# microsoft/Sora

Measured on AMD Instinct MI355X. Metric: IQ Msamples/s through 802.11a 54 Mbps RX PHY, higher is better.
Workload: dtype int16 IQ / u8 path metrics

## Files before the change

### sora_amd/csrc/k_scan.hip

```cpp
#include <hip/hip_runtime.h>
#include "kernels.h"

namespace sora {

constexpr uint32_t kRing = 512;
__shared__ uint32_t s_ring[kRing];

#ifdef SORA_SCAN_PROBE
__device__ unsigned long long g_scan_probe[16];
#define PROBE_DECL() long long _pa[8] = {0, 0, 0, 0, 0, 0, 0, 0}; unsigned _pn[8] = {0, 0, 0, 0, 0, 0, 0, 0}
#define PROBE_T0() const long long _t0 = clock64()
#define PROBE_ADD(i) do { _pa[i] += clock64() - _t0; _pn[i]++; } while (0)
#define PROBE_T(n) const long long n = clock64()
#define PROBE_A(n, i) do { _pa[i] += clock64() - n; _pn[i]++; } while (0)
#define PROBE_TK() const long long _tk = clock64()
#define PROBE_ADDK(i) do { _pa[i] += clock64() - _tk; _pn[i]++; \
    if (blockIdx.x == 0 && threadIdx.x == 0) for (int q = 0; q < 8; q++) { g_scan_probe[q] += (unsigned long long)_pa[q]; g_scan_probe[8 + q] += _pn[q]; } } while (0)
#else
#define PROBE_DECL()
#define PROBE_T0()
#define PROBE_ADD(i)
#define PROBE_T(n)
#define PROBE_A(n, i)
#define PROBE_TK()
#define PROBE_ADDK(i)
#endif

struct Acc4 { int reg; uint32_t Z; };
__device__ __forceinline__ void acc_clear(Acc4& a) { a.reg = 0; a.Z = 0; }
__device__ __forceinline__ void acc_push(Acc4& a, int d)
{
    const int e0 = __builtin_amdgcn_readfirstlane((int)a.Z);
    a.reg = (int)((unsigned)a.reg + (unsigned)d - (unsigned)e0);
    const uint32_t sh = (uint32_t)__builtin_amdgcn_update_dpp(0, (int)a.Z, 0x104, 0xF, 0xF, true);
    a.Z = (threadIdx.x & 12u) == 12u ? (uint32_t)d : sh;
}
__device__ __forceinline__ uint32_t group_scan(uint32_t t)
{
    t += (uint32_t)__builtin_amdgcn_update_dpp(0, (int)t, 0x114, 0xF, 0xF, true);
    t += (uint32_t)__builtin_amdgcn_update_dpp(0, (int)t, 0x118, 0xF, 0xF, true);
    t += (uint32_t)__builtin_amdgcn_update_dpp(0, (int)t, 0x142, 0xA, 0xF, false);
    return t;
}

__device__ __forceinline__ uint32_t group_scan64(uint32_t t)
{
    t += (uint32_t)__builtin_amdgcn_update_dpp(0, (int)t, 0x114, 0xF, 0xF, true);
    t += (uint32_t)__builtin_amdgcn_update_dpp(0, (int)t, 0x118, 0xF, 0xF, true);
    t += (uint32_t)__builtin_amdgcn_update_dpp(0, (int)t, 0x142, 0xA, 0xF, false);
    t += (uint32_t)__builtin_amdgcn_update_dpp(0, (int)t, 0x143, 0xC, 0xF, false);
    return t;
}
__device__ __forceinline__ uint32_t shift16(uint32_t v, uint32_t first)
{
    auto r16 = __builtin_amdgcn_permlane16_swap(v, v, false, false);
    auto r32 = __builtin_amdgcn_permlane32_swap(r16[1], r16[1], false, false);
    const uint32_t l = threadIdx.x;
    return l < 16u ? first : (l & 48u) == 32u ? r32[0] : r16[0];
}
__device__ __forceinline__ uint32_t compress4(uint64_t x)
{
    x = (x | (x >> 3)) & 0x0303030303030303ull;
    x = (x | (x >> 6)) & 0x000F000F000F000Full;
    x = (x | (x >> 12)) & 0x000000FF000000FFull;
    return (uint32_t)((x | (x >> 24)) & 0xFFFFull);
}

template <int CTRL> __device__ __forceinline__ unsigned sdpp(unsigned v) { return (unsigned)__builtin_amdgcn_update_dpp(0, (int)v, CTRL, 0xF, 0xF, true); }
__device__ __forceinline__ unsigned quad_sum(unsigned v) { v += sdpp<0xB1>(v); v += sdpp<0x4E>(v); return v; }
__device__ __forceinline__ unsigned row_sum(unsigned v) { v = quad_sum(v); v += sdpp<0x141>(v); v += sdpp<0x140>(v); return v; }
__device__ __forceinline__ unsigned other_row_even(unsigned v)
{
    auto r = __builtin_amdgcn_permlane16_swap(v, v, false, false);
    return r[0];
}
__device__ __forceinline__ int wave_sum(int v)
{
    unsigned u = row_sum((unsigned)v);
    auto r16 = __builtin_amdgcn_permlane16_swap(u, u, false, false);
    u = r16[0] + r16[1];
    auto r32 = __builtin_amdgcn_permlane32_swap(u, u, false, false);
    return (int)(r32[0] + r32[1]);
}
__device__ __forceinline__ unsigned wave_min(unsigned v)
{
    v = min(v, sdpp<0xB1>(v)); v = min(v, sdpp<0x4E>(v)); v = min(v, sdpp<0x141>(v)); v = min(v, sdpp<0x140>(v));
    auto r16 = __builtin_amdgcn_permlane16_swap(v, v, false, false);
    v = min(r16[0], r16[1]);
    auto r32 = __builtin_amdgcn_permlane32_swap(v, v, false, false);
    return min(r32[0], r32[1]);
}

__device__ __constant__ uint8_t kLtsSeq[64] = {
    0,1,0,0,1,1,0,1,0,1,0,0,0,0,0,1, 1,0,0,1,0,1,0,1,1,1,1,0,0,0,0,0,
    0,0,0,0,0,0,1,1,0,0,1,1,0,1,0,1, 1,1,1,1,1,0,0,1,1,0,1,0,1,1,1,1 };

__device__ __forceinline__ int carrier_bin(int k)
{
    if (k < 24) { int b = 38 + k; if (b >= 43) b++; if (b >= 57) b++; return b; }
    int b = 1 + (k - 24); if (b >= 7) b++; if (b >= 21) b++; return b;
}

struct ScanTabs { const short* uatan2; const uint32_t* rot; const uint8_t* demap; const uint16_t* deint; const uint32_t* tw64; const uint32_t* tw16; };
template <typename P> __device__ __forceinline__ P* uni_ptr(P* p)
{
    const uint64_t v = (uint64_t)(uintptr_t)p;
    const uint32_t lo = (uint32_t)__builtin_amdgcn_readfirstlane((int)(uint32_t)v), hi = (uint32_t)__builtin_amdgcn_readfirstlane((int)(uint32_t)(v >> 32));
    return (P*)(uintptr_t)(((uint64_t)hi << 32) | lo);
}
__device__ __forceinline__ Tables tables_of(const ScanTabs& b)
{
    Tables T = {};
    T.uatan2 = uni_ptr(b.uatan2); T.rot = uni_ptr(b.rot); T.demap = uni_ptr(b.demap); T.deint = uni_ptr(b.deint); T.tw64 = uni_ptr(b.tw64); T.tw16 = uni_ptr(b.tw16);
    return T;
}

struct SigOut { uint32_t ok, kbps, len, nsym, cr, nb; int cfo_comp, sfo_comp, cfo_tr, sfo_tr, cfo; };
__device__ __noinline__ SigOut header_section(ScanTabs tabs, uint32_t lts_start_, FrameCtx* fx_)
{
    const Tables T = tables_of(tabs);
    FrameCtx* fx = uni_ptr(fx_);
    const uint32_t lts_start = (uint32_t)__builtin_amdgcn_readfirstlane((int)lts_start_), sym_start = lts_start + 144u;
    __shared__ uint32_t s_a[64], s_b[64];
    __shared__ uint8_t  s_soft[64];
    const int lane = threadIdx.x, e = lane & 15;
    auto sync = []() { wave_lds_sync(); };
    const Fft64TwPk W = fft64_twiddles_pk(T, e);
    const int t2 = lane < 24 ? 2 * lane : 0;
    const int d0 = T.deint[t2], d1 = T.deint[t2 + 1];
    const cpx x1 = sra(unpack(s_ring[(lts_start + 8u + (uint32_t)lane) & (kRing - 1u)]), 1);
    const cpx x2 = unpack(s_ring[(lts_start + 72u + (uint32_t)lane) & (kRing - 1u)]);
    const cpx sg = sra(unpack(s_ring[(sym_start + 8u + (uint32_t)lane) & (kRing - 1u)]), 1);
    int re, im; conj_mul32(x2, x1, re, im);
    const int sum_re = __builtin_amdgcn_readfirstlane(wave_sum(re >> 5)), sum_im = __builtin_amdgcn_readfirstlane(wave_sum(im >> 5));
    const int arg = __builtin_amdgcn_readfirstlane(uatan2(T, sum_im, sum_re));
    const int cfo = arg >> 6;
    const cpx fc = rot_coeff(T, w16(lane * cfo));
    fx->freq[lane] = pack(fc);
    s_a[lane] = pack(mul_q15(x1, fc));
    s_b[lane] = pack(mul_q15(sg, fc));
    {
        uint32_t* const sf = (lane & 16) ? s_b : s_a;
        sync();
        const pcx xin[4] = { sf[e], sf[e + 16], sf[e + 32], sf[e + 48] };
        fft64_core_pk(xin, sf, e, W, sync);
    }
    const unsigned slot = __brev((unsigned)lane) >> 26;
    const cpx Yl = unpack(s_a[slot]), Ys = unpack(s_b[slot]);
    cpx eq = mk(0, 0);
    {
        uint32_t coef = 0;
        if (!(lane >= 28 && lane < 36)) {
            const int en = sqnorm(Yl) >> 8;
            const cpx L = mk(kLtsSeq[lane] ? 1600 : -1600, 0);
            int cre, cim; conj_mul32(L, Yl, cre, cim);
            int rre = 0, rim = 0;
            if (en != 0) { rre = cre / en; rim = cim / en; }
            coef = pack(mk(w16(rre), w16(rim)));
            int qr, qi; mul32(Ys, unpack(coef), qr, qi);
            eq = mk(w16(qr >> 8), w16(qi >> 8));
        }
        fx->chan[lane] = coef;
    }
    const cpx pc = mul_q15(eq, mk(0x7fff, 0));
    const uint32_t ppc = pack(pc);
    const cpx p43 = unpack((uint32_t)__builtin_amdgcn_readlane((int)ppc, 43)), p57 = unpack((uint32_t)__builtin_amdgcn_readlane((int)ppc, 57));
    const cpx p7 = unpack((uint32_t)__builtin_amdgcn_readlane((int)ppc, 7)), p21 = unpack((uint32_t)__builtin_amdgcn_readlane((int)ppc, 21));
    const int th1 = __builtin_amdgcn_readfirstlane(uatan2(T, p43.im, p43.re)), th2 = __builtin_amdgcn_readfirstlane(uatan2(T, p57.im, p57.re));
    const int th3 = __builtin_amdgcn_readfirstlane(uatan2(T, p7.im, p7.re)),   th4 = __builtin_amdgcn_readfirstlane(uatan2(T, -p21.im, -p21.re));
    const int avg = w16((th1 + th2 + th3 + th4) / 4);
    const int del = w16(((th3 - th1) / 28 + (th4 - th2) / 28) >> 1);
    const int cfo_tracker = w16(avg >> 2), sfo_tracker = w16(del >> 2);
    const int cfo_comp = w16(avg + cfo_tracker), sfo_comp = w16(del + sfo_tracker);
    {
        const int cidx = lane < 32 ? lane : lane - 64;
        const cpx r = mul_q15(pc, rot_coeff(T, w16(avg + cidx * del)));
        int v = r.re >> 4; v = min(max(v, -128), 127);
        s_soft[lane] = (uint8_t)((v >= -30) + (v >= -17) + (v >= -8) + (v >= 0) + (v >= 9) + (v >= 18) + (v >= 31));
    }
    sync();
    uint8_t sa = 0, sb = 0;
    if (lane < 24) { sa = s_soft[carrier_bin(d0)]; sb = s_soft[carrier_bin(d1)]; }
    auto rol6c = [](unsigned x, unsigned k) { return ((x << k) | (x >> (6u - k))) & 63u; };
    int selV[6], negV[6], n29V[6];
#pragma unroll
    for (int k = 0; k < 6; k++) {
        const unsigned n = k ? rol6c((unsigned)lane, (unsigned)k) : (unsigned)lane;
        const int cA = __popc(n & 0155) & 1, cB = __popc(n & 0117) & 1;
        selV[k] = (cA ^ cB) ? -1 : 0; negV[k] = cB ? -1 : 0; n29V[k] = cB ? 29 : 0;
    }
    unsigned m = (lane == 0) ? 0u : 0x30u;
    uint64_t dec[25];
    dec[0] = 0;
#pragma unroll
    for (int u = 1; u <= 24; u++) {
        const int ph = (u - 1) % 6, k = u % 6;
        const unsigned X = 32u >> ph;
        unsigned pm;
        if (ph == 0) { auto r = __builtin_amdgcn_permlane32_swap(m, m, false, false); pm = lane < 32 ? r[1] : r[0]; }
        else if (ph == 1) { auto r = __builtin_amdgcn_permlane16_swap(m, m, false, false); pm = (lane & 16) ? r[0] : r[1]; }
        else if (ph == 2) pm = sdpp<0x128>(m);
        else if (ph == 3) {
            const int t4 = __builtin_amdgcn_update_dpp(0, (int)m, 0x114, 0xF, 0xA, false);
            pm = (unsigned)__builtin_amdgcn_update_dpp(t4, (int)m, 0x104, 0xF, 0x5, false);
        }
        else if (ph == 4) pm = sdpp<0x4E>(m);
        else pm = sdpp<0xB1>(m);
        asm volatile("" : "+v"(pm));
        const bool own_hi = ((unsigned)lane & X) != 0u;
        const unsigned m0 = own_hi ? pm : m, m1 = own_hi ? m : pm;
        const int va = __builtin_amdgcn_readlane((int)sa, u - 1), vb = __builtin_amdgcn_readlane((int)sb, u - 1);
        const int P = 2 * va + 2 * vb, dQP = 14 - 4 * va;
        const int x = P + (selV[k] & dQP);
        const unsigned b0 = (unsigned)((x ^ negV[k]) + n29V[k]), b1 = 28u - b0;
        const unsigned c0 = (m0 + b0) & 0xFE, c1 = ((m1 + b1) & 0xFF) | 1;
        m = min(c0, c1);
        dec[u] = __ballot(m & 1);
        if ((u & 7) == 0) m = (m - (wave_min(m) & 0xFE)) & 0xFF;
    }
    const unsigned key = (m << 8) | ((unsigned)lane << 2);
    const unsigned kmin = (unsigned)__builtin_amdgcn_readfirstlane((int)wave_min(key));
    int pos = (int)((kmin >> 2) & 0x3F) | (int)(((kmin >> 8) & 1) << 6);
    uint32_t sig = 0;
#pragma unroll
    for (int b = 0; b < 24; b++) {
        sig |= (uint32_t)((pos >> 6) & 1) << (23 - b);
        pos = (pos >> 1) & 0x3F;
        const unsigned r = (unsigned)(23 - b) % 6u;
        const unsigned ln = r ? rol6c((unsigned)pos, 6u - r) : (unsigned)pos;
        pos |= (int)((dec[23 - b] >> ln) & 1) << 6;
    }
    sig = (uint32_t)__builtin_amdgcn_readfirstlane((int)sig) >> 6;
    bool ok = true;
    sig &= 0xFFFFFF;
    if (sig & 0xFC0010) ok = false;
    uint32_t par = (sig >> 16) ^ sig; par = (par >> 8) ^ par; par = (par >> 4) ^ par; par = (par >> 2) ^ par; par = (par >> 1) ^ par;
    if (par & 1) ok = false;
    uint32_t kbps = 0; int nd = 0, nb = 0, cr = 0;
    switch (sig & 0xF) {
    case 0x8: kbps = 48000; nd = 192; nb = 6; cr = 1; break;  case 0x9: kbps = 24000; nd = 96;  nb = 4; cr = 0; break;
    case 0xA: kbps = 12000; nd = 48;  nb = 2; cr = 0; break;  case 0xB: kbps = 6000;  nd = 24;  nb = 1; cr = 0; break;
    case 0xC: kbps = 54000; nd = 216; nb = 6; cr = 2; break;  case 0xD: kbps = 36000; nd = 144; nb = 4; cr = 2; break;
    case 0xE: kbps = 18000; nd = 72;  nb = 2; cr = 2; break;  case 0xF: kbps = 9000;  nd = 36;  nb = 1; cr = 2; break;
    default: ok = false; break;
    }
    const uint32_t len = (sig >> 5) & 0xFFF;
    if (len > 2500) ok = false;
    SigOut O;
    O.ok = ok ? 1u : 0u; O.kbps = kbps; O.len = len; O.cr = (uint32_t)cr; O.nb = (uint32_t)nb;
    O.nsym = ok ? (len * 8 + 16 + 6 + (uint32_t)nd - 1) / (uint32_t)nd : 0u;
    O.cfo_comp = cfo_comp; O.sfo_comp = sfo_comp; O.cfo_tr = cfo_tracker; O.sfo_tr = sfo_tracker; O.cfo = cfo;
    __threadfence_block();
    sync();
    return O;
}

constexpr uint32_t kContMagic = 0x534F5241u;
__device__ __noinline__ void cont_store(uint32_t* crec, uint32_t* consumed, uint32_t Hv, uint32_t Zr, uint32_t Zi, uint32_t Ze, int rr, int ri, int re,
                                        uint32_t sense_count, uint32_t high_count, int peak_corr, int peak_index, uint32_t dc_cnt, int sum_dc_re, int sum_dc_im,
                                        int dc_re, int dc_im, uint32_t at, uint32_t nfr)
{
    const int l = threadIdx.x;
    const uint32_t zr = (uint32_t)__shfl((int)Zr, 4 * (l & 3)), zi = (uint32_t)__shfl((int)Zi, 4 * (l & 3)), ze = (uint32_t)__shfl((int)Ze, 4 * (l & 3));
    const uint32_t hv = (uint32_t)__shfl((int)Hv, l & 15);
    uint32_t v = l < 16 ? hv : l < 20 ? zr : l < 24 ? zi : l < 28 ? ze : 0u;
    const uint32_t sc[16] = { (uint32_t)rr, (uint32_t)ri, (uint32_t)re, sense_count, high_count, (uint32_t)peak_corr, (uint32_t)peak_index, dc_cnt,
                              (uint32_t)sum_dc_re, (uint32_t)sum_dc_im, (uint32_t)dc_re, (uint32_t)dc_im, at, kContMagic, nfr, 0u };
#pragma unroll
    for (int k = 0; k < 16; k++) if (l == 28 + k) v = sc[k];
    crec[l] = v;
    if (l == 0) *consumed = at;
}
__device__ __noinline__ void cont_rows(const uint32_t* crec, uint32_t* nframes, FrameRow* rows, uint32_t written)
{
    const uint32_t n = (uint32_t)__builtin_amdgcn_readlane((int)crec[threadIdx.x], 42);
    if (threadIdx.x == 0) {
        *nframes = n;
        for (uint32_t k = n; k < written; k++) rows[k].valid = 0;
    }
}

__device__ __forceinline__ uint32_t div14(uint32_t x) { return (uint32_t)(((uint64_t)x * 0x92492493ull) >> 35); }
__device__ __forceinline__ uint32_t call_end(uint32_t burst_end) { return div14(burst_end + 13u) * 14u; }

__global__ void __launch_bounds__(64, 4) k_scan(ScanArgs A)
{
    const uint32_t cap_i = blockIdx.x;
    if (cap_i >= A.ncaps) return;
    const int lane = threadIdx.x;
    const CapDesc cd = A.caps[cap_i];
    const uint32_t* iq = A.iq + cd.offset;
    const uint32_t sh = A.str - 1u;
    const uint32_t NS = (cd.nsamples / (14u << sh)) * 14u;
    const Tables& T = A.T;
    const ScanTabs tabs = { T.uatan2, T.rot, T.demap, T.deint, T.tw64, T.tw16 };

    uint32_t n0 = 0, n1 = 0, n2 = 0, n3 = 0, r_lo = 0, r_hi = 0;
    auto issue = [&](uint32_t base) {
        const uint32_t i = base + (uint32_t)lane;
        n0 = i < NS ? iq[(size_t)i << sh] : 0u;
        n1 = i + 64u < NS ? iq[(size_t)(i + 64u) << sh] : 0u;
        n2 = i + 128u < NS ? iq[(size_t)(i + 128u) << sh] : 0u;
        n3 = i + 192u < NS ? iq[(size_t)(i + 192u) << sh] : 0u;
    };
    auto aim = [&](uint32_t at) { if (at < r_lo || at >= r_hi + 256u) { r_lo = r_hi = at; issue(at); } };
    auto fill = [&](uint32_t at, uint32_t len) {
        aim(at);
        while (at + len > r_hi) {
            const uint32_t w = r_hi + (uint32_t)lane;
            s_ring[w & (kRing - 1u)] = n0; s_ring[(w + 64u) & (kRing - 1u)] = n1; s_ring[(w + 128u) & (kRing - 1u)] = n2; s_ring[(w + 192u) & (kRing - 1u)] = n3;
            r_hi += 256u;
            if (r_hi - r_lo > kRing) r_lo = r_hi - kRing;
            issue(r_hi);
        }
    };
    issue(0);

    if (A.own_slots && A.slot_row) for (uint32_t i = (uint32_t)lane; i < cd.nslots; i += 64u) A.slot_row[cd.slot_base + i] = 0xFFFFFFFFu;
    if (cap_i == 0) {
        if (A.zero_a) for (uint32_t i = (uint32_t)lane; i < A.nzero_a; i += 64u) A.zero_a[i] = 0u;
        if (A.zero_b) for (uint32_t i = (uint32_t)lane; i < A.nzero_b; i += 64u) A.zero_b[i] = 0u;
    }
    const uint32_t chk0 = T.sts[lane & 15], chk1 = T.sts[16 + (lane & 15)], chk2 = T.sts[32 + (lane & 15)], chk3 = T.sts[48 + (lane & 15)];
    const uint32_t est_base = (uint32_t)(lane >> 2) * 16u + 4u * (uint32_t)(lane & 3);
    const uint32_t est0 = T.sts[est_base], est1 = T.sts[est_base + 1], est2 = T.sts[est_base + 2], est3 = T.sts[est_base + 3];

    uint32_t Hv = 0;
    Acc4 ac_re, ac_im, energy;
    uint32_t auto_count = 0, sense_count = 0, high_count = 0; int sync_high = 0, peak_corr = 0, peak_index = 0;
    uint32_t dc_cnt = 8; int sum_dc_re = 0, sum_dc_im = 0;
    int dc_re = 0, dc_im = 0;
    int cca_detected = 0;
    uint32_t frame_start = 0, nfr = 0;
    bool to_pending = false; uint32_t pend_end = 0;

    auto cs_reset = [&]() {
        Hv = 0;
        acc_clear(ac_re); acc_clear(ac_im); acc_clear(energy);
        auto_count = sense_count = high_count = 0; sync_high = 0; peak_corr = 0; peak_index = 0;
        dc_cnt = 8; sum_dc_re = sum_dc_im = 0;
    };
    cs_reset();

    const bool streaming = A.cont != nullptr;
    auto cont_save = [&](uint32_t at) {
        cont_store(A.cont + (size_t)cap_i * kContWords, A.consumed + cap_i, Hv, ac_re.Z, ac_im.Z, energy.Z, ac_re.reg, ac_im.reg, energy.reg, sense_count,
                high_count, peak_corr, peak_index,
                   dc_cnt, sum_dc_re, sum_dc_im, dc_re, dc_im, at << sh, nfr);
    };
    if (streaming) {
        if (lane == 0) A.consumed[cap_i] = 0;
        const uint32_t v = A.cont[(size_t)cap_i * kContWords + lane];
        if (lane == 42) A.cont[(size_t)cap_i * kContWords + lane] = 0;
        if ((uint32_t)__builtin_amdgcn_readlane((int)v, 41) == kContMagic) {
            auto sc = [&](int k) { return (uint32_t)__builtin_amdgcn_readlane((int)v, 28 + k); };
            Hv = (uint32_t)__shfl((int)v, lane & 15);
            ac_re.Z = (uint32_t)__shfl((int)v, 16 + ((lane & 15) >> 2)); ac_im.Z = (uint32_t)__shfl((int)v, 20 + ((lane & 15) >> 2));
                energy.Z = (uint32_t)__shfl((int)v, 24 + ((lane & 15) >> 2));
            ac_re.reg = (int)sc(0); ac_im.reg = (int)sc(1); energy.reg = (int)sc(2); sense_count = sc(3); high_count = sc(4); peak_corr = (int)sc(5); peak_index = (int)sc(6);
            dc_cnt = sc(7); sum_dc_re = (int)sc(8); sum_dc_im = (int)sc(9); dc_re = (int)sc(10); dc_im = (int)sc(11);
        }
    }

    uint32_t q_job = 0, nq = 0;
    auto flush_jobs = [&]() {
        if (nq == 0) return;
        const bool have = (uint32_t)lane < nq;
        const uint32_t cr = q_job >> 28, row = q_job & 0x0FFFFFFFu;
        const uint64_t m0 = __ballot(have && cr == 0u), m1 = __ballot(have && cr == 1u), m2 = __ballot(have && cr == 2u);
        const uint32_t cnt = lane == 0 ? (uint32_t)__popcll(m0) : lane == 1 ? (uint32_t)__popcll(m1) : (uint32_t)__popcll(m2);
        uint32_t base = 0;
        if (lane < 3 && cnt) base = atomicAdd(A.njobs + lane, cnt);
        const uint32_t b0 = (uint32_t)__builtin_amdgcn_readlane((int)base, 0), b1 = (uint32_t)__builtin_amdgcn_readlane((int)base, 1), b2 = (uint32_t)__builtin_amdgcn_readlane((int)base, 2);
        if (have) {
            const uint64_t mine = cr == 0u ? m0 : cr == 1u ? m1 : m2, below = ((uint64_t)1 << lane) - 1u;
            A.joblist[(size_t)cr * A.nrows + (cr == 0u ? b0 : cr == 1u ? b1 : b2) + (uint32_t)__popcll(mine & below)] = row;
        }
        nq = 0;
    };
    uint32_t s = 0;
    PROBE_DECL();
    PROBE_TK();
    auto ctx_of = [&](uint32_t k) { return A.fctx + (k < A.max_frames ? (size_t)cap_i * A.max_frames + k : (size_t)A.nrows + cap_i); };
    auto uni = [](int v) { return __builtin_amdgcn_readfirstlane(v); };

    for (;;) {
        PROBE_T(_tg);
        if (to_pending && s + 4u > pend_end) {
            to_pending = false; cca_detected = 0; cs_reset();
        }
        if (s + 4u > NS) break;
        if (!sync_high) {
            const bool plain = !to_pending && auto_count == 0;
            const uint32_t p = dc_cnt;
            uint32_t K = min(min((NS - s) >> 2, p + 9u), 16u);
            uint32_t jraise = 0xFFFFu, ce_raise = 0;
            if (to_pending) K = min(K, (pend_end - s) >> 2);
            else {
                jraise = sense_count >= 84u ? 0u : (84u - sense_count + 3u) / 4u - 1u;
                if (jraise < K) { const uint32_t be = s + 4u * jraise + 4u; ce_raise = call_end(be); K = min(K, jraise + 1u + ((ce_raise - be) >> 2)); }
            }
            if (streaming) {
                if (A.keep_queue) {
                    const uint32_t m = s % 140u;
                    if (m == 0u && plain) cont_save(s);
                    if (m) K = min(K, (143u - m) >> 2);
                } else {
                    const uint32_t m = s - div14(s) * 14u;
                    if (m == 0u && plain) cont_save(s);
                    const uint32_t j = (3u * (m >> 1)) % 7u;
                    K = min(K, j ? j : 7u);
                }
            }
            PROBE_A(_tg, 1);
            PROBE_T0();
            fill(s, 64u);
            const cpx x = unpack(s_ring[(s + (uint32_t)lane) & (kRing - 1u)]);
            int dcr = dc_re, dci = dc_im;
            if (p + 1u < K) {
                const unsigned hr = group_scan64(quad_sum((unsigned)(w16(x.re - dc_re) >> 5))), hi_ = group_scan64(quad_sum((unsigned)(w16(x.im - dc_im) >> 5)));
                const int sr = w16(sum_dc_re + __builtin_amdgcn_readlane((int)hr, (int)(4u * p))), si = w16(sum_dc_im + __builtin_amdgcn_readlane((int)hi_, (int)(4u * p)));
                const int d1r = w16(dc_re + (sr >> 2)), d1i = w16(dc_im + (si >> 2));
                const bool behind = (uint32_t)lane > 4u * p + 3u;
                dcr = behind ? d1r : dc_re; dci = behind ? d1i : dc_im;
            }
            const cpx pi = mk(w16(x.re - dcr), w16(x.im - dci));
            const cpx pii = sra(pi, 2);
            const uint32_t ppk = pack(pii);
            const uint32_t prev = shift16(ppk, Hv);
            int re, im; conj_mul32(pii, unpack(prev), re, im);
            unsigned vr = (unsigned)(re >> 4), vi = (unsigned)(im >> 4), ve = (unsigned)(sqnorm(pii) >> 4);
            vr = quad_sum(vr); vi = quad_sum(vi); ve = quad_sum(ve);
            const uint32_t Dr = group_scan64(quad_sum((unsigned)(pi.re >> 5))), Di = group_scan64(quad_sum((unsigned)(pi.im >> 5)));
            const uint32_t Rr = (uint32_t)ac_re.reg + group_scan64(vr - shift16(vr, ac_re.Z)), Ri = (uint32_t)ac_im.reg + group_scan64(vi - shift16(vi, ac_im.Z)),
                           Re = (uint32_t)energy.reg + group_scan64(ve - shift16(ve, energy.Z));
            const int iAuto_v = abs((int)Rr) + abs((int)Ri), iEnergy_v = (int)Re;
            const bool carrier = iEnergy_v > (int)A.thr && iAuto_v >= iEnergy_v - (iEnergy_v >> 3);
            const uint32_t hits = compress4((uint64_t)__ballot(carrier) & 0x1111111111111111ull) & ((1u << K) - 1u);
            const uint32_t a = min(auto_count, 3u);
            const uint32_t M = (hits << a) | ((1u << a) - 1u);
            const uint32_t run = M & (M >> 1) & (M >> 2) & (M >> 3);
            const bool est = run != 0;
            const uint32_t done = est ? (uint32_t)__builtin_ctz(run) + 4u - a : K;
            const uint32_t bits = (1u << done) - 1u;
            const uint32_t th = hits & bits;
            if (est) auto_count = 4;
            else {
                const uint32_t inv = ~th & bits;
                auto_count = inv ? done - 1u - (31u - (uint32_t)__builtin_clz(inv)) : min(auto_count + done, 4u);
            }
            if (!to_pending && jraise < min(th ? (uint32_t)__builtin_ctz(th) : done, done)) { to_pending = true; pend_end = ce_raise; }
            sense_count = th ? 4u * (done - 1u - (31u - (uint32_t)__builtin_clz(th))) : sense_count + 4u * done;
            {
                const int last = (int)(4u * (done - 1u));
                ac_re.reg = __builtin_amdgcn_readlane((int)Rr, last); ac_im.reg = __builtin_amdgcn_readlane((int)Ri, last); energy.reg = __builtin_amdgcn_readlane((int)Re, last);
                const uint32_t src = ((uint32_t)lane & 15u) + 4u * done;
                const int from_old = (int)(((uint32_t)lane & 48u) | (src & 15u)), from_new = (int)(src - 16u);
                const uint32_t fr = (uint32_t)__shfl((int)vr, from_new), fi = (uint32_t)__shfl((int)vi, from_new), fe = (uint32_t)__shfl((int)ve, from_new);
                const uint32_t fresh = (uint32_t)__shfl((int)ppk, from_new);
                if (done < 4u) {
                    const bool old = src < 16u;
                    const uint32_t kr = (uint32_t)__shfl((int)ac_re.Z, from_old), ki = (uint32_t)__shfl((int)ac_im.Z, from_old), ke = (uint32_t)__shfl((int)energy.Z, from_old);
                    const uint32_t keep = (uint32_t)__shfl((int)Hv, from_old);
                    ac_re.Z = old ? kr : fr; ac_im.Z = old ? ki : fi; energy.Z = old ? ke : fe; Hv = old ? keep : fresh;
                } else { ac_re.Z = fr; ac_im.Z = fi; energy.Z = fe; Hv = fresh; }
            }
            s += 4u * done;
            PROBE_ADD(3);
            if (est) {
                PROBE_T0();
                unsigned sr = 0, si = 0;
                {
                    const int q4 = 4 * (lane & 3);
                    const uint32_t h0 = (uint32_t)__shfl((int)Hv, q4), h1 = (uint32_t)__shfl((int)Hv, q4 + 1), h2 = (uint32_t)__shfl((int)Hv, q4 + 2), h3 = (uint32_t)__shfl((int)Hv, q4 + 3);
                    int cr_, ci_;
                    conj_mul32(unpack(est0), unpack(h0), cr_, ci_); sr += (unsigned)cr_; si += (unsigned)ci_;
                    conj_mul32(unpack(est1), unpack(h1), cr_, ci_); sr += (unsigned)cr_; si += (unsigned)ci_;
                    conj_mul32(unpack(est2), unpack(h2), cr_, ci_); sr += (unsigned)cr_; si += (unsigned)ci_;
                    conj_mul32(unpack(est3), unpack(h3), cr_, ci_); sr += (unsigned)cr_; si += (unsigned)ci_;
                }
                sr = quad_sum(sr); si = quad_sum(si);
                const int corr = abs((int)sr) + abs((int)si);
                int sum_corr = 0, best = 0, best_i = 0;
#pragma unroll
                for (int p = 0; p < 16; p++) {
                    const int cp = __builtin_amdgcn_readlane(corr, 4 * p);
                    if (cp > best) { best = cp; best_i = p; }
                    sum_corr += cp;
                }
                peak_corr = best; if (best > 0) peak_index = best_i;
                if (peak_corr > (sum_corr >> 3)) {
                    sync_high = 1; high_count = 0;
                    if (peak_index > 3) { high_count = (uint32_t)peak_index / 4; peak_index &= 3; }
                }
                PROBE_ADD(0);
            }
            const uint32_t ndc = done - (sync_high ? 1u : 0u);
            if (ndc > p) {
                const int at_p = __builtin_amdgcn_readlane((int)Dr, (int)(4u * p)), at_pi = __builtin_amdgcn_readlane((int)Di, (int)(4u * p));
                dc_re = w16(dc_re + (w16(sum_dc_re + at_p) >> 2)); dc_im = w16(dc_im + (w16(sum_dc_im + at_pi) >> 2));
                const uint32_t n1 = ndc - 1u - p;
                const int lastd = (int)(4u * (ndc - 1u));
                const int seg_re = w16(__builtin_amdgcn_readlane((int)Dr, lastd) - at_p), seg_im = w16(__builtin_amdgcn_readlane((int)Di, lastd) - at_pi);
                if (n1 == 8u) { dc_re = w16(dc_re + (seg_re >> 2)); dc_im = w16(dc_im + (seg_im >> 2)); sum_dc_re = sum_dc_im = 0; dc_cnt = 7; }
                else { sum_dc_re = seg_re; sum_dc_im = seg_im; dc_cnt = 7u - n1; }
            } else if (ndc) {
                const int lastd = (int)(4u * (ndc - 1u));
                sum_dc_re = w16(sum_dc_re + __builtin_amdgcn_readlane((int)Dr, lastd));
                sum_dc_im = w16(sum_dc_im + __builtin_amdgcn_readlane((int)Di, lastd));
                dc_cnt -= ndc;
            }
            continue;
        }

        {
            PROBE_T0();
            const uint32_t o = high_count & 3u;
            uint32_t Kn = min(16u - o, (NS - s) >> 2);
            if (to_pending) Kn = min(Kn, (pend_end - s) >> 2);
            fill(s, 64u);
            const cpx x = unpack(s_ring[(s + (uint32_t)lane - 4u * o) & (kRing - 1u)]);
            const cpx pi = mk(w16(x.re - dc_re), w16(x.im - dc_im));
            const uint32_t ppk = pack(sra(pi, 2));
            uint32_t hvr = Hv;
            if (o == 1u) hvr = sdpp<0x124>(Hv); else if (o == 2u) hvr = sdpp<0x128>(Hv); else if (o == 3u) hvr = sdpp<0x12C>(Hv);
            const uint32_t c = (uint32_t)lane < 4u * o ? hvr : ppk;
            const uint32_t pat = peak_index == 0 ? chk0 : peak_index == 1 ? chk1 : peak_index == 2 ? chk2 : chk3;
            int re, im; conj_mul32(unpack(pat), unpack(c), re, im);
            const unsigned ur = row_sum((unsigned)re), ui = row_sum((unsigned)im);
            unsigned dr = (unsigned)(pi.re >> 5), di = (unsigned)(pi.im >> 5);
            dr = quad_sum(dr); di = quad_sum(di);
            const uint32_t nchk = (o + Kn) >> 2;
            uint32_t taken = Kn;
#pragma unroll
            for (uint32_t r = 0; r < 4u; r++) {
                if (r < nchk && taken == Kn) {
                    const int corr = abs(__builtin_amdgcn_readlane((int)ur, 16 * (int)r)) + abs(__builtin_amdgcn_readlane((int)ui, 16 * (int)r));
                    if (corr < (peak_corr >> 1)) {
                        const uint32_t b = 4u * (r + 1u) - o - 1u;
                        taken = b + 1u;
                        if (high_count + taken > 8u) { cca_detected = 1; frame_start = s + 4u * b + 4u; }
                        else {
                            sync_high = 0; sense_count = 0;
                            sum_dc_re = w16(sum_dc_re + w16(__builtin_amdgcn_readlane((int)dr, 16 * (int)r + 12)));
                            sum_dc_im = w16(sum_dc_im + w16(__builtin_amdgcn_readlane((int)di, 16 * (int)r + 12)));
                            if (dc_cnt == 0) {
                                dc_re = w16(dc_re + (sum_dc_re >> 2)); dc_im = w16(dc_im + (sum_dc_im >> 2));
                                dc_cnt = 8; sum_dc_re = sum_dc_im = 0;
                            }
                            dc_cnt--;
                        }
                        if (taken == Kn) break;
                    } else if (corr > peak_corr) peak_corr = corr;
                }
            }
            high_count += taken;
            {
                const uint32_t src = ((uint32_t)lane & 15u) + 4u * taken;
                const uint32_t fresh = (uint32_t)__shfl((int)ppk, (int)((src - 16u + 4u * o) & 63u));
                if (taken < 4u) { const uint32_t keep = (uint32_t)__shfl((int)Hv, (int)(((uint32_t)lane & 48u) | (src & 15u))); Hv = src < 16u ? keep : fresh; }
                else Hv = fresh;
            }
            s += 4u * taken;
            PROBE_ADD(4);
        }
        if (!cca_detected) continue;

        const uint32_t lts_start = s, sym_start = s + 144u;
        if (sym_start + 80u > NS) break;
        PROBE_T(_tf);
        fill(lts_start, 224u);
        PROBE_A(_tf, 6);
        FrameCtx* const fx = ctx_of(nfr);
        PROBE_T(_ts);
        const SigOut so = header_section(tabs, lts_start, fx);
        const int r_cfo = uni(so.cfo);
        PROBE_A(_ts, 2);
        PROBE_T(_tc);
        const bool ok = uni((int)so.ok) != 0;
        const uint32_t r_nsym = ok ? (uint32_t)uni((int)so.nsym) : 0u, r_cr = ok ? (uint32_t)uni((int)so.cr) : 0u;
        const uint64_t ev = ok ? (uint64_t)sym_start + 80ull * (r_nsym + 1u) : (uint64_t)sym_start + 80ull;
        if (ev > NS) break;
        const uint32_t ce = call_end((uint32_t)ev), consumed_to = (uint32_t)ev + (((ce - (uint32_t)ev) >> 2) << 2);
        const uint32_t s_next = A.keep_queue ? consumed_to : ce;
        aim(s_next);
        {
            const bool has_row = nfr < A.max_frames;
            const uint32_t slot0 = cd.slot_base + sym_start / 80u;
            if (ok && has_row) {
                if ((uint32_t)lane == nq) q_job = (r_cr << 28) | (cap_i * A.max_frames + nfr);
                if (++nq == 64u) flush_jobs();
                if (A.slot_row) for (uint32_t sy = 1u + (uint32_t)lane; sy <= r_nsym; sy += 64u) A.slot_row[slot0 + sy] = cap_i * A.max_frames + nfr;
            }
            if (lane == 0 && has_row) {
                FrameRow row;
                row.capture = cap_i; row.start_sample = frame_start; row.end_sample = ok ? (uint32_t)ev : consumed_to;
                row.error_code = ok ? 0u : E_PLCP_HEADER_FAIL;
                row.rate_kbps = ok ? (uint32_t)uni((int)so.kbps) : 0u; row.length = (uint16_t)(ok ? (uint32_t)uni((int)so.len) : 0u); row.nsym = (uint16_t)r_nsym;
                row.code_rate = (uint16_t)r_cr; row.nbpsc = (uint16_t)(ok ? (uint32_t)uni((int)so.nb) : 0u); row.slot0 = slot0; row.crc32 = 0;
                row.cfo_est = (int16_t)r_cfo; row.cfo_comp = (int16_t)uni(so.cfo_comp); row.sfo_comp = (int16_t)uni(so.sfo_comp);
                row.cfo_tracker = (int16_t)uni(so.cfo_tr); row.sfo_tracker = (int16_t)uni(so.sfo_tr); row.valid = 1;
                row.data_start = sym_start; row.pad[0] = row.pad[1] = row.pad[2] = 0;
                A.frames[(size_t)cap_i * A.max_frames + nfr] = row;
            }
        }
        nfr++;
        s = s_next;
        to_pending = false; cca_detected = 0; cs_reset();
        PROBE_A(_tc, 7);
    }
    if (streaming && s == NS && !cca_detected && !sync_high && auto_count == 0 && !to_pending && (!A.keep_queue || s % 140u == 0u)) cont_save(s);
    flush_jobs();
    if (streaming) cont_rows(A.cont + (size_t)cap_i * kContWords, A.nframes + cap_i, A.frames + (size_t)cap_i * A.max_frames, min(nfr, A.max_frames));
    else if (lane == 0) A.nframes[cap_i] = nfr;
    PROBE_ADDK(5);
}

}

#ifdef SORA_SCAN_PROBE
extern "C" __attribute__((visibility("default"))) int sora_debug_scan_probe(unsigned long long* out, int reset)
{
    if (hipMemcpyFromSymbol(out, HIP_SYMBOL(sora::g_scan_probe), sizeof(unsigned long long) * 16) != hipSuccess) return -1;
    if (reset) { unsigned long long z[16] = {0}; (void)hipMemcpyToSymbol(HIP_SYMBOL(sora::g_scan_probe), z, sizeof(z)); }
    return 0;
}
#endif
```

Baseline: 55090.

## Restructure SIGNAL Viterbi ACS with packed branch metrics and table-driven selectors

```diff
diff --git a/sora_amd/csrc/k_scan.hip b/sora_amd/csrc/k_scan.hip
--- a/sora_amd/csrc/k_scan.hip
+++ b/sora_amd/csrc/k_scan.hip
@@ -115,6 +115,22 @@
     return T;
 }
 
+struct SigSel { uint32_t w[64][8]; };
+constexpr SigSel make_sig_sel()
+{
+    SigSel t = {};
+    for (unsigned p = 0; p < 64; p++)
+        for (unsigned k = 0; k < 6; k++) {
+            const unsigned n = k ? ((p << k) | (p >> (6u - k))) & 63u : p;
+            unsigned a = n & 0155u, b = n & 0117u, cA = 0, cB = 0;
+            for (; a; a >>= 1) cA ^= a & 1u;
+            for (; b; b >>= 1) cB ^= b & 1u;
+            t.w[p][k] = ((cA + 2u * cB) << 24) | 0x000C0C0Cu;
+        }
+    return t;
+}
+__device__ __constant__ const SigSel kSigSel = make_sig_sel();
+
 struct SigOut { uint32_t ok, kbps, len, nsym, cr, nb; int cfo_comp, sfo_comp, cfo_tr, sfo_tr, cfo; };
 __device__ __noinline__ SigOut header_section(ScanTabs tabs, uint32_t lts_start_, FrameCtx* fx_)
 {
@@ -128,6 +144,9 @@
     const Fft64TwPk W = fft64_twiddles_pk(T, e);
     const int t2 = lane < 24 ? 2 * lane : 0;
     const int d0 = T.deint[t2], d1 = T.deint[t2 + 1];
+    unsigned sel[6];
+#pragma unroll
+    for (int k = 0; k < 6; k++) sel[k] = kSigSel.w[lane][k];
     const cpx x1 = sra(unpack(s_ring[(lts_start + 8u + (uint32_t)lane) & (kRing - 1u)]), 1);
     const cpx x2 = unpack(s_ring[(lts_start + 72u + (uint32_t)lane) & (kRing - 1u)]);
     const cpx sg = sra(unpack(s_ring[(sym_start + 8u + (uint32_t)lane) & (kRing - 1u)]), 1);
@@ -181,56 +200,50 @@
     sync();
     uint8_t sa = 0, sb = 0;
     if (lane < 24) { sa = s_soft[carrier_bin(d0)]; sb = s_soft[carrier_bin(d1)]; }
-    auto rol6c = [](unsigned x, unsigned k) { return ((x << k) | (x >> (6u - k))) & 63u; };
-    int selV[6], negV[6], n29V[6];
-#pragma unroll
-    for (int k = 0; k < 6; k++) {
-        const unsigned n = k ? rol6c((unsigned)lane, (unsigned)k) : (unsigned)lane;
-        const int cA = __popc(n & 0155) & 1, cB = __popc(n & 0117) & 1;
-        selV[k] = (cA ^ cB) ? -1 : 0; negV[k] = cB ? -1 : 0; n29V[k] = cB ? 29 : 0;
-    }
-    unsigned m = (lane == 0) ? 0u : 0x30u;
+    const unsigned bmw = [&]() {
+        const unsigned P = 2u * sa + 2u * sb, Q = 14u - 2u * sa + 2u * sb;
+        return P | (Q << 8) | ((28u - Q) << 16) | ((28u - P) << 24);
+    }();
+    unsigned M = (lane == 0) ? 0u : 0x30u << 24;
     uint64_t dec[25];
-    dec[0] = 0;
+    bool last = false;
 #pragma unroll
     for (int u = 1; u <= 24; u++) {
         const int ph = (u - 1) % 6, k = u % 6;
-        const unsigned X = 32u >> ph;
-        unsigned pm;
-        if (ph == 0) { auto r = __builtin_amdgcn_permlane32_swap(m, m, false, false); pm = lane < 32 ? r[1] : r[0]; }
-        else if (ph == 1) { auto r = __builtin_amdgcn_permlane16_swap(m, m, false, false); pm = (lane & 16) ? r[0] : r[1]; }
-        else if (ph == 2) pm = sdpp<0x128>(m);
+        unsigned M0, M1;
+        if (ph == 0) { auto r = __builtin_amdgcn_permlane32_swap(M, M, false, false); M0 = r[0]; M1 = r[1]; }
+        else if (ph == 1) { auto r = __builtin_amdgcn_permlane16_swap(M, M, false, false); M0 = r[0]; M1 = r[1]; }
+        else if (ph == 2) {
+            M0 = (unsigned)__builtin_amdgcn_update_dpp((int)M, (int)M, 0x118, 0xF, 0xC, false);
+            M1 = (unsigned)__builtin_amdgcn_update_dpp((int)M, (int)M, 0x108, 0xF, 0x3, false);
+        }
         else if (ph == 3) {
-            const int t4 = __builtin_amdgcn_update_dpp(0, (int)m, 0x114, 0xF, 0xA, false);
-            pm = (unsigned)__builtin_amdgcn_update_dpp(t4, (int)m, 0x104, 0xF, 0x5, false);
-        }
-        else if (ph == 4) pm = sdpp<0x4E>(m);
-        else pm = sdpp<0xB1>(m);
-        asm volatile("" : "+v"(pm));
-        const bool own_hi = ((unsigned)lane & X) != 0u;
-        const unsigned m0 = own_hi ? pm : m, m1 = own_hi ? m : pm;
-        const int va = __builtin_amdgcn_readlane((int)sa, u - 1), vb = __builtin_amdgcn_readlane((int)sb, u - 1);
-        const int P = 2 * va + 2 * vb, dQP = 14 - 4 * va;
-        const int x = P + (selV[k] & dQP);
-        const unsigned b0 = (unsigned)((x ^ negV[k]) + n29V[k]), b1 = 28u - b0;
-        const unsigned c0 = (m0 + b0) & 0xFE, c1 = ((m1 + b1) & 0xFF) | 1;
-        m = min(c0, c1);
-        dec[u] = __ballot(m & 1);
-        if ((u & 7) == 0) m = (m - (wave_min(m) & 0xFE)) & 0xFF;
-    }
-    const unsigned key = (m << 8) | ((unsigned)lane << 2);
-    const unsigned kmin = (unsigned)__builtin_amdgcn_readfirstlane((int)wave_min(key));
-    int pos = (int)((kmin >> 2) & 0x3F) | (int)(((kmin >> 8) & 1) << 6);
+            M0 = (unsigned)__builtin_amdgcn_update_dpp((int)M, (int)M, 0x114, 0xF, 0xA, false);
+            M1 = (unsigned)__builtin_amdgcn_update_dpp((int)M, (int)M, 0x104, 0xF, 0x5, false);
+        }
+        else if (ph == 4) { M0 = sdpp<0x44>(M); M1 = sdpp<0xEE>(M); }
+        else { M0 = sdpp<0xA0>(M); M1 = sdpp<0xF5>(M); }
+        asm volatile("" : "+v"(M0), "+v"(M1));
+        const unsigned w = (unsigned)__builtin_amdgcn_readlane((int)bmw, u - 1);
+        const unsigned B0 = __builtin_amdgcn_perm(w, w, sel[k]);
+        const unsigned C0 = M0 + B0, C1 = M1 + ((28u << 24) - B0);
+        last = C1 < C0;
+        dec[u] = __ballot(last);
+        M = min(C0, C1);
+        if (u == 8 || u == 16) M -= wave_min(M);
+    }
+    const unsigned key = M | (last ? 1u << 24 : 0u) | (unsigned)lane;
+    unsigned L = (unsigned)__builtin_amdgcn_readfirstlane((int)wave_min(key)) & 63u;
     uint32_t sig = 0;
 #pragma unroll
-    for (int b = 0; b < 24; b++) {
-        sig |= (uint32_t)((pos >> 6) & 1) << (23 - b);
-        pos = (pos >> 1) & 0x3F;
-        const unsigned r = (unsigned)(23 - b) % 6u;
-        const unsigned ln = r ? rol6c((unsigned)pos, 6u - r) : (unsigned)pos;
-        pos |= (int)((dec[23 - b] >> ln) & 1) << 6;
-    }
-    sig = (uint32_t)__builtin_amdgcn_readfirstlane((int)sig) >> 6;
+    for (int g = 0; g < 3; g++) {
+#pragma unroll
+        for (int i = 0; i < 6; i++) {
+            const unsigned d = (unsigned)(dec[24 - 6 * g - i] >> L) & 1u;
+            L = (L & ~(1u << i)) | (d << i);
+        }
+        sig |= __brev(L) >> (14 + 6 * g);
+    }
     bool ok = true;
     sig &= 0xFFFFFF;
     if (sig & 0xFC0010) ok = false;
@@ -383,13 +396,14 @@
     PROBE_TK();
     auto ctx_of = [&](uint32_t k) { return A.fctx + (k < A.max_frames ? (size_t)cap_i * A.max_frames + k : (size_t)A.nrows + cap_i); };
     auto uni = [](int v) { return __builtin_amdgcn_readfirstlane(v); };
+    const uint32_t need = streaming ? 4u : 224u;
 
     for (;;) {
         PROBE_T(_tg);
         if (to_pending && s + 4u > pend_end) {
             to_pending = false; cca_detected = 0; cs_reset();
         }
-        if (s + 4u > NS) break;
+        if (s + need > NS) break;
         if (!sync_high) {
             const bool plain = !to_pending && auto_count == 0;
             const uint32_t p = dc_cnt;
```

Measured after the change: 56090, median of 6. 1.8% higher.
